# angelocatalani/neural-network-compression

Measured on AMD Instinct MI355X. Metric: weights/sec through prune+k-means (K=256), higher is better.
Workload: dtype f32

## Files before the change

### include/nnc.h

```cpp
#ifndef NNC_H
#define NNC_H

#include <stddef.h>
#include <stdint.h>

#ifdef __cplusplus
extern "C" {
#endif

#define NNC_VERSION 100

#define NNC_OK 0
#define NNC_EINVAL (-1)
#define NNC_ENOSPACE (-2)
#define NNC_EHIP (-3)
#define NNC_ENODEV (-4)

#define NNC_KMAX 1040
#define NNC_CHUNK 8192

int nnc_version(void);
const char *nnc_last_error(void);
int nnc_device_info(char *arch_out, size_t arch_len, int *cu_count_out);

// ... 118 lines not shown

int nnc_kmeans_assign(const float *x, void *ws, const nnc_kmeans_params *p, int which, void *labels_out,
                      int label_bytes, float *quant_out, float *dist_out, int64_t *dist_hist4096_dev, void *stream);

int nnc_topm_hist_f32(const float *d, int64_t n, int32_t shift, int32_t width, int32_t prefix_shift, uint32_t prefix,
                      int64_t *hist4096_dev, void *stream);
int nnc_topm_compact_f32(const float *d, const float *x, int64_t n, uint32_t thr_bits, int64_t *keys_dev,
                         int64_t cap, int64_t *count_dev, void *stream);

int nnc_kmeans_relocate(void *ws, const int64_t *keys_sorted_dev, int32_t nkeys, void *stream);

int nnc_kmeans_reloc_candidates(const float *x_sorted, void *ws, const nnc_kmeans_params *p, int32_t window,
                                float *cand_x_dev, int64_t cap, void *win_dev, int32_t *meta_dev, void *stream);
int nnc_kmeans_relocate_checked(void *ws, const float *cand_x_dev, const float *cand_d_dev, const void *win_dev,
                                const int32_t *meta_dev, int32_t n_empty, int64_t *keys_out_dev, void *stream);
int32_t nnc_kmeans_reloc_window(int64_t n, int32_t n_empty);
size_t nnc_kmeans_reloc_scratch_bytes(int32_t k, int32_t window);
int nnc_kmeans_relocate_windowed(const float *x_sorted, void *ws, const nnc_kmeans_params *p, int32_t n_empty,
                                 void *scratch_dev, size_t scratch_bytes, void *stream);
int nnc_kmeans_reloc_select_local(const float *x_sorted, void *ws, const nnc_kmeans_params *p, int32_t n_empty,
                                  void *scratch_dev, size_t scratch_bytes, int64_t *keys_out_dev, void *stream);
int32_t *nnc_kmeans_reloc_flag(void *ws);
int nnc_kmeans_relocate_if_proven(void *ws, const int64_t *keys_sorted_dev, int32_t nkeys, void *stream);
int nnc_labels_equal(const void *a, const void *b, int64_t n, int label_bytes, int32_t *flag_dev, void *stream);
int nnc_ref_sums_f32(const float *x, int64_t n, float x_mean, const void *labels, int32_t label_bytes, int32_t k,
                     float *sums_out_dev, int64_t *counts_out_dev, void *stream);
int nnc_kmeans_set_done_if(void *ws, const int32_t *flag_dev, int32_t done_code, void *stream);

int nnc_bincount(const void *labels, int label_bytes, int64_t n, int32_t k, int64_t *counts_dev, void *stream);

// ... 343 lines not shown
```

### neural_network_compression_amd/_native.py

```python
from __future__ import annotations

import ctypes
import os

from . import build as _build

c_void_p = ctypes.c_void_p
c_int = ctypes.c_int
c_i32 = ctypes.c_int32
c_i64 = ctypes.c_int64
c_f32 = ctypes.c_float
c_size = ctypes.c_size_t

NNC_OK = 0
NNC_KMAX = 1040
NNC_CHUNK = 8192
FOLD_SUM, FOLD_MEAN, FOLD_STD = 0, 1, 2
NNC_KM_TWO_LAUNCH = 1
NNC_KM_LOOP = 2
NNC_KM_MASS_IN_PLACE = 4
NNC_KM_LOOP_KMAX = 64
CBMM_NONE, CBMM_STREAM, CBMM_TILED, CBMM_BIAS = 0, 1, 2, 3
CBMM_PLAN_LEN = 12
CBMM_PLAN_FIELDS = ("path", "vb", "mt", "copies", "entries", "splits", "rps", "aligned", "lds", "col_tiles", "row_tiles", "workspace")
# ... 126 lines not shown
    "nnc_kmeans_status_async": (c_int, [c_void_p, ctypes.POINTER(KMeansStatus), c_void_p]),
    "nnc_kmeans_status_publish": (c_int, [c_void_p, c_void_p, ctypes.c_uint64, c_void_p]),
    "nnc_kmeans_iterate_publish": (c_int, [c_void_p, c_void_p, ctypes.POINTER(KMeansParams), c_i32, c_void_p, ctypes.c_uint64, c_void_p]),
    "nnc_kmeans_fit": (c_int, [c_void_p, c_void_p, ctypes.POINTER(KMeansParams), c_i32, c_i32, c_void_p, c_size, c_void_p,
                               ctypes.POINTER(ctypes.c_uint64), ctypes.POINTER(KMeansStatus), ctypes.POINTER(c_i32), c_void_p]),
    "nnc_kmeans_fit_sharded": (c_int, [c_void_p, c_void_p, c_void_p, ctypes.POINTER(KMeansParams), ctypes.c_int64, c_i32, c_i32, c_void_p, c_size,
                                       c_void_p, ctypes.POINTER(ctypes.c_uint64), ctypes.POINTER(KMeansStatus), ctypes.POINTER(c_i32), c_void_p]),
    "nnc_kmeans_set_done": (c_int, [c_void_p, c_i32, c_void_p]),
    "nnc_kmeans_label_counts": (c_int, [c_void_p, c_void_p, ctypes.POINTER(KMeansParams), c_int, c_void_p, c_void_p]),
    "nnc_kmeans_get_centers": (c_int, [c_void_p, c_int, c_int, c_void_p, c_void_p]),
    "nnc_kmeans_assign": (c_int, [c_void_p, c_void_p, ctypes.POINTER(KMeansParams), c_int, c_void_p, c_int, c_void_p, c_void_p, c_void_p, c_void_p]),
    "nnc_topm_hist_f32": (c_int, [c_void_p, c_i64, c_i32, c_i32, c_i32, ctypes.c_uint32, c_void_p, c_void_p]),
    "nnc_topm_compact_f32": (c_int, [c_void_p, c_void_p, c_i64, ctypes.c_uint32, c_void_p, c_i64, c_void_p, c_void_p]),
    "nnc_kmeans_relocate": (c_int, [c_void_p, c_void_p, c_i32, c_void_p]),
    "nnc_kmeans_reloc_candidates": (c_int, [c_void_p, c_void_p, ctypes.POINTER(KMeansParams), c_i32, c_void_p, c_i64, c_void_p, c_void_p, c_void_p]),
    "nnc_kmeans_relocate_checked": (c_int, [c_void_p, c_void_p, c_void_p, c_void_p, c_void_p, c_i32, c_void_p, c_void_p]),
    "nnc_kmeans_reloc_window": (c_i32, [c_i64, c_i32]),
    "nnc_kmeans_reloc_scratch_bytes": (c_size, [c_i32, c_i32]),
    "nnc_kmeans_relocate_windowed": (c_int, [c_void_p, c_void_p, ctypes.POINTER(KMeansParams), c_i32, c_void_p, c_size, c_void_p]),
    "nnc_kmeans_reloc_select_local": (c_int, [c_void_p, c_void_p, ctypes.POINTER(KMeansParams), c_i32, c_void_p, c_size, c_void_p, c_void_p]),
    "nnc_kmeans_reloc_flag": (c_void_p, [c_void_p]),
    "nnc_kmeans_relocate_if_proven": (c_int, [c_void_p, c_void_p, c_i32, c_void_p]),
    "nnc_labels_equal": (c_int, [c_void_p, c_void_p, c_i64, c_int, c_void_p, c_void_p]),
    "nnc_ref_sums_f32": (c_int, [c_void_p, c_i64, ctypes.c_float, c_void_p, c_i32, c_i32, c_void_p, c_void_p, c_void_p]),
    "nnc_kmeans_set_done_if": (c_int, [c_void_p, c_void_p, c_i32, c_void_p]),
    "nnc_bincount": (c_int, [c_void_p, c_int, c_i64, c_i32, c_void_p, c_void_p]),
    "nnc_kmeans_fit_reference_f32": (c_int, [c_void_p, c_i32, c_void_p, c_i32, c_i32, c_f32, c_void_p, c_void_p, c_void_p, c_void_p, c_void_p, c_void_p]),
    "nnc_compress_layer_workspace_bytes": (c_size, [c_i64, c_i32]),
    "nnc_compress_layer_host_bytes": (c_size, []),
    "nnc_compress_layer_f32": (c_int, [c_void_p, c_i64, ctypes.POINTER(LayerParams), c_void_p, c_void_p, c_void_p, c_void_p, c_size, c_void_p, c_size,
# ... 182 lines not shown
```

### neural_network_compression_amd/csrc/nnc_hip.hip

```cpp
#include "nnc_common.hpp"
#include "nnc_km_shared.hpp"


extern "C" size_t nnc_kmeans_workspace_bytes(int32_t k)
{
    (void)k;
    return sizeof(KmWs) + 256;
}

extern "C" int32_t nnc_fix_shift(float absmax, int64_t n_total)
{
    int L = 1;
    while (((int64_t)1 << L) < n_total && L < 62) L++;
    if (!(absmax > 0.0f) || !std::isfinite(absmax)) return 0;
    int P = 0;
    (void)std::frexp((double)absmax, &P);
    return std::min(28, 62 - L) - P;
}

__device__ __forceinline__ int fix_f32(float v, int Sft)
{
    return (int)rintf(ldexpf(v, Sft));
}

// ... 2623 lines not shown
#ifndef KM_RELOC_WMIN
#define KM_RELOC_WMIN 64
#endif
#define KM_SURV_MAX 2048
#define KM_SURV_SMALL 384

__device__ __forceinline__ bool km_spec_decide(const KmWs *__restrict__ ws, long long n, int spec_wmax, int *W_out)
{
    const int done = ws->st.done, paused = ws->st.paused, it = ws->st.iter, same = ws->st.same_counts, ne = ws->st.n_empty;
    long long w = KM_RELOC_WMIN;
    while (w < ne) w *= 2;
    if (W_out) *W_out = (int)w;
    return !done && paused == 1 && !(it >= 1 && same) && ne >= 1 && w <= spec_wmax && 2 * w <= n;
}

__device__ __forceinline__ void km_reloc_windows_body(const float *__restrict__ xs, long long n, KmWs *__restrict__ ws, int W, long long cap,
                                                      KmWin *__restrict__ win, int *__restrict__ meta, unsigned *__restrict__ hist0, int spec_wmax)
{
    if (spec_wmax > 0) {
        const bool go = km_spec_decide(ws, n, spec_wmax, &W);
        if (threadIdx.x == 0) ws->spec_go = go ? 1 : 0;
        if (!go) return;
    }
    if (hist0) for (int i = threadIdx.x; i < 4096; i += KM_THREADS) hist0[i] = 0u;
    __shared__ long long bnd[2 * KM_THREADS + 2];
    __shared__ long long wst[2 * KM_THREADS], wen[2 * KM_THREADS];
    __shared__ long long wave_tot[KM_THREADS / 64];
    const int tid = threadIdx.x;
    const KmTab *tab = &ws->tab[ws->cur];
    const int kt = tab->ku, k = ws->p.k;
    const float mean = ws->p.x_mean;
    const int i0 = 2 * tid, i1 = 2 * tid + 1;
    long long a0 = (i0 < kt) ? ws->partials_local[k + tab->orig[i0]] : 0;
    long long a1 = (i1 < kt) ? ws->partials_local[k + tab->orig[i1]] : 0;
    block_scan2<false>(a0, a1, wave_tot);
    if (tid == 0) bnd[0] = 0;
    bnd[i0 + 1] = a0; bnd[i1 + 1] = a1;
    __syncthreads();
    const int nwin = kt + 1;
    const int bad = (bnd[kt] != n) ? 1 : 0;
    if (bad) {
        for (int j = tid; j < nwin; j += KM_THREADS) { KmWin w; w.start = 0; w.len = 0; w.off = 0; win[j] = w; }
        if (tid == 0) { meta[0] = 0; meta[1] = nwin; meta[2] = 1; meta[3] = W; }
        return;
    }
    for (int j = tid; j < 2 * KM_THREADS; j += KM_THREADS) {
        long long st = 0, en = 0;
        if (j < nwin) {
            long long b = bnd[j];
            b = b < 0 ? 0 : (b > n ? n : b);
            long long wl = W, wr = W;
            if (j > 0 && j < kt && n > 0) {
                const double zr = tab->zr[j - 1], zl = tab->zl[j];
                bool more_r = true, more_l = true;
                while (more_r || more_l) {
                    const long long pr = b + wr - 1, pl = b - wl;
                    const float vr = (more_r && pr < n - 1) ? xs[pr] : 0.0f;
                    const float vl = (more_l && pl > 0) ? xs[pl] : 0.0f;
// ... 5 lines not shown
            en = b + wr > n ? n : b + wr;
        }
        wst[j] = st; wen[j] = en;
    }
    __syncthreads();
    long long e0 = wen[i0], e1 = wen[i1];
    block_scan2<true>(e0, e1, wave_tot);
    if (tid == 0) bnd[0] = 0;
    bnd[i0 + 1] = e0; bnd[i1 + 1] = e1;
    __syncthreads();
    long long l0 = 0, l1 = 0, s0 = 0, s1 = 0;
    if (i0 < nwin) { s0 = wst[i0] > bnd[i0] ? wst[i0] : bnd[i0]; l0 = bnd[i0 + 1] - s0; if (l0 <= 0) { l0 = 0; s0 = bnd[i0 + 1]; } }
    if (i1 < nwin) { s1 = wst[i1] > bnd[i1] ? wst[i1] : bnd[i1]; l1 = bnd[i1 + 1] - s1; if (l1 <= 0) { l1 = 0; s1 = bnd[i1 + 1]; } }
    const long long len0 = l0, len1 = l1;
    block_scan2<false>(l0, l1, wave_tot);
    if (i0 < nwin) { KmWin w; w.start = s0; w.len = (int)len0; w.off = l0 <= cap ? (int)(l0 - len0) : 0; win[i0] = w; }
    if (i1 < nwin) { KmWin w; w.start = s1; w.len = (int)len1; w.off = l1 <= cap ? (int)(l1 - len1) : 0; win[i1] = w; }
    if (tid == (nwin - 1) / 2) {
        const long long total = ((nwin - 1) & 1) ? l1 : l0;
        const int over = total > cap ? 1 : 0;
        meta[0] = over ? 0 : (int)total; meta[1] = nwin; meta[2] = bad | over; meta[3] = W;
    }
}

__global__ __launch_bounds__(KM_THREADS) void k_reloc_windows(const float *__restrict__ xs, long long n, KmWs *__restrict__ ws,
                                                              int W, long long cap, KmWin *__restrict__ win, int *__restrict__ meta,
                                                              unsigned *__restrict__ hist0 = nullptr, int spec_wmax = 0)
{
    if (spec_wmax > 0 && threadIdx.x == 0 && km_spec_decide(ws, n, spec_wmax, nullptr)) ws->tab[ws->cur].n_ovf = 0;
    km_reloc_windows_body(xs, n, ws, W, cap, win, meta, hist0, spec_wmax);
}

__global__ __launch_bounds__(KM_THREADS) void k_reloc_head(const float *__restrict__ xs, long long n, KmWs *__restrict__ ws, long long cap,
                                                           KmWin *__restrict__ win, int *__restrict__ meta, unsigned *__restrict__ hist0, int spec_wmax)
{
    if (blockIdx.x == gridDim.x - 1) {
// ... 75 lines not shown
        float xc[1];
        int p[1];
        km_resolve<1>(c, xv, xc, p);
        const float dd = xc[0] - cval_s[p[0]];
        const float dv = dd * dd;
        cand_x[i] = xv[0];
        cand_d[i] = dv;
        atomicAdd(&h0_s[(__float_as_uint(dv) >> 19) & 4095u], 1u);
    }
    __syncthreads();
    for (int i = threadIdx.x; i < 4096; i += KM_THREADS)
        if (h0_s[i]) atomicAdd(&hist0[i], h0_s[i]);
    if (blockIdx.x == 0 && threadIdx.x < 4 && total + threadIdx.x < cap) { cand_x[total + threadIdx.x] = 0.0f; cand_d[total + threadIdx.x] = 0.0f; }
}

__device__ __forceinline__ void km_reloc_select_body(KmWs *__restrict__ ws, const float *__restrict__ cand_x,
                                                     const float *__restrict__ cand_d, const KmWin *__restrict__ win,
                                                     const int *__restrict__ meta, int n_empty, long long *__restrict__ keys_out,
                                                     int do_relocate, const unsigned *__restrict__ hist0, int spec)
{
    if (spec) {
        if (!ws->spec_go) return;
        n_empty = ws->st.n_empty;
    }
    __shared__ __align__(8) unsigned hist[4096];
    __shared__ unsigned long long surv[KM_SURV_MAX];
    __shared__ int wave_i[KM_THREADS / 64];
    __shared__ int s_cut, s_above, s_ge, s_nsurv, s_bad;
    __shared__ KmRelocLds rl;
    __shared__ double zl_s[NNC_KMAX];
    const int tid = threadIdx.x, lane = tid & 63, wv = tid >> 6;
    unsigned long long *strc = NNC_KM_TRACE_PTR;
#define RSTAMP(i) do { if (strc && tid == 0) strc[7000 + (i)] = __builtin_amdgcn_s_memrealtime(); } while (0)
    RSTAMP(0);
    const int n_cand = meta[0];
    const int n_empty_ws = do_relocate ? km_relocate_prepare(ws, &rl) : 0;
    {
        int bad0 = meta[2] ? 1 : 0;
        if (n_empty < 1 || n_cand < n_empty) bad0 |= 2;
        if (bad0) { if (tid == 0) { ws->reloc_fail = bad0; if (spec) ws->st.n_unproven += 1; } return; }
    }
    const int nvec = n_cand >> 2;
    const uint4 *d4 = reinterpret_cast<const uint4 *>(cand_d);
    unsigned prefix = 0, thr = 0;
    int pshift = -1, above = 0, total_ge = n_cand;
    const int shifts[3] = {19, 7, 0}, widths[3] = {12, 12, 7};
    for (int lvl = 0; lvl < 3; lvl++) {
        const int shift = shifts[lvl], width = widths[lvl];
        const unsigned mask = (1u << width) - 1u;
        for (int i = tid; i < 4096; i += KM_THREADS) hist[i] = (lvl == 0 && hist0) ? hist0[i] : 0u;
        if (tid == 0) { s_cut = 0; s_above = above; s_ge = total_ge; }
        __syncthreads();
        const unsigned NOBIN = 0xFFFFu;
        auto bin_of = [&](unsigned u) -> unsigned { return (pshift < 0 || (u >> pshift) == prefix) ? ((u >> shift) & mask) : NOBIN; };
        for (int v0 = 0; v0 < ((lvl == 0 && hist0) ? 0 : nvec); v0 += 8 * KM_THREADS) {
            uint4 qv[8];
#pragma unroll
            for (int u = 0; u < 8; u++) {
                const int v = v0 + u * KM_THREADS + tid;
                qv[u] = v < nvec ? d4[v] : make_uint4(0u, 0u, 0u, 0u);
            }
#pragma unroll
            for (int u = 0; u < 8; u++) {
                const int v = v0 + u * KM_THREADS + tid;
                const bool have = v < nvec;
// ... 158 lines not shown
    __syncthreads();
    RSTAMP(4);
    const int any_bad = s_bad;
    if (tid == 0) { ws->reloc_fail = any_bad; if (spec && any_bad) ws->st.n_unproven += 1; }
    if (any_bad || !do_relocate) return;
    __threadfence_block();
    km_relocate_apply(ws, keys_out, min(m, n_empty + 1), n_empty_ws, &rl);
    if (spec && tid == 0) ws->st.n_relocated += 1;
    RSTAMP(5);
#undef RSTAMP
}

__global__ __launch_bounds__(KM_THREADS) void k_reloc_select(KmWs *__restrict__ ws, const float *__restrict__ cand_x,
                                                             const float *__restrict__ cand_d, const KmWin *__restrict__ win,
                                                             const int *__restrict__ meta, int n_empty, long long *__restrict__ keys_out,
                                                             int do_relocate, const unsigned *__restrict__ hist0, int spec)
{
    km_reloc_select_body(ws, cand_x, cand_d, win, meta, n_empty, keys_out, do_relocate, hist0, spec);
}

__global__ __launch_bounds__(KM_THREADS) void k_reloc_select_finalize(KmWs *__restrict__ ws, const float *__restrict__ cand_x,
                                                                      const float *__restrict__ cand_d, const KmWin *__restrict__ win,
                                                                      const int *__restrict__ meta, long long *__restrict__ keys_out,
                                                                      const unsigned *__restrict__ hist0, nnc_kmeans_status *host_st,
                                                                      unsigned long long *host_ticket, unsigned long long ticket, int lazy)
{
    km_reloc_select_body(ws, cand_x, cand_d, win, meta, 0, keys_out, 1, hist0, 1);
    __syncthreads();
    __builtin_amdgcn_fence(__ATOMIC_ACQUIRE, "agent");
    km_finalize_kernel<KM_THREADS, false, false>(ws, FIN_FROM_PARTIALS, 2, host_st, host_ticket, ticket, lazy, nullptr, 0);
}

static std::atomic<int> g_reloc_dist_attr[NNC_MAX_DEVICES];
static int km_reloc_windows_dist(const float *x_sorted, void *ws, const nnc_kmeans_params *p, int32_t window, float *cand_x,
                                 float *cand_d, int64_t cap, void *win_dev, int32_t *meta_dev, unsigned *hist0, void *stream)
{
    int glog2, rlog2;
    km_defaults(p, &glog2, &rlog2);
    const size_t lds = km_lds_bytes(p->k, glog2, rlog2, false) + (NNC_KMAX + 2) * sizeof(int);
// ... 23 lines not shown
    int rc = km_check(ws, p, "nnc_kmeans_reloc_candidates");
    if (rc) return rc;
    if (!x_sorted || !cand_x_dev || !win_dev || !meta_dev || window < 1) return fail(NNC_EINVAL, "nnc_kmeans_reloc_candidates: bad argument");
    if (cap < 2 * (int64_t)window * (p->k + 1) || cap > 0x7FFFFFFF) return fail(NNC_ENOSPACE, "nnc_kmeans_reloc_candidates: cap must be in [2 * window * (k + 1), 2^31)");
    NNC_LAUNCH_PROF(NNC_PROF_RELOC, k_reloc_windows, dim3(1), dim3(KM_THREADS), 0, S(stream), x_sorted, (long long)p->n,
                       reinterpret_cast<KmWs *>(ws), (int)window, (long long)cap,
                       reinterpret_cast<KmWin *>(win_dev), reinterpret_cast<int *>(meta_dev), (unsigned *)nullptr, 0);
    LAUNCHCHK("k_reloc_windows");
    const int grid = (int)std::min<int64_t>(256, (cap + 16383) / 16384 + p->k / 4 + 1);
    hipLaunchKernelGGL(k_reloc_fill, dim3(grid), dim3(256), 0, S(stream), x_sorted, reinterpret_cast<const KmWin *>(win_dev),
                       reinterpret_cast<const int *>(meta_dev), cand_x_dev, (long long)cap);
    LAUNCHCHK("k_reloc_fill");
    return NNC_OK;
}

#ifdef NNC_DIAG
extern "C" int nnc_debug_reloc_fail(void *ws, int32_t *host_out)
{
    if (!ws || !host_out) return fail(NNC_EINVAL, "nnc_debug_reloc_fail: null pointer");
    HIPCHK(hipMemcpy(host_out, &reinterpret_cast<KmWs *>(ws)->reloc_fail, sizeof(int32_t), hipMemcpyDeviceToHost));
    return NNC_OK;
}
#endif

extern "C" int nnc_kmeans_relocate_checked(void *ws, const float *cand_x_dev, const float *cand_d_dev, const void *win_dev,
                                           const int32_t *meta_dev, int32_t n_empty, int64_t *keys_out_dev, void *stream)
{
    if (!ws || !cand_x_dev || !cand_d_dev || !win_dev || !meta_dev || !keys_out_dev || n_empty < 1 || n_empty > NNC_KMAX)
        return fail(NNC_EINVAL, "nnc_kmeans_relocate_checked: bad argument");
    NNC_LAUNCH_PROF(NNC_PROF_RELOC, k_reloc_select, dim3(1), dim3(KM_THREADS), 0, S(stream), reinterpret_cast<KmWs *>(ws), cand_x_dev, cand_d_dev,
                       reinterpret_cast<const KmWin *>(win_dev), reinterpret_cast<const int *>(meta_dev), (int)n_empty,
                       reinterpret_cast<long long *>(keys_out_dev), 1, (const unsigned *)nullptr, 0);
    LAUNCHCHK("k_reloc_select");
    return NNC_OK;
}


extern "C" int32_t nnc_kmeans_reloc_window(int64_t n, int32_t n_empty)
{
    int64_t w = KM_RELOC_WMIN;
    while (w < n_empty) w *= 2;
    if (n_empty < 1 || w > 1024 || 2 * w > n) return 0;
    return (int32_t)w;
}

static int64_t reloc_cap(int32_t k, int32_t window) { return 8 * (int64_t)window * (k + 1); }

// ... 13 lines not shown
    if (window == 0) return fail(NNC_EINVAL, "nnc_kmeans_relocate_windowed: not applicable (nnc_kmeans_reloc_window() == 0)");
    if (!x_sorted || !scratch_dev || (reinterpret_cast<uintptr_t>(scratch_dev) & 255) != 0)
        return fail(NNC_EINVAL, "nnc_kmeans_relocate_windowed: null or unaligned (256 B) pointer");
    if (scratch_bytes < nnc_kmeans_reloc_scratch_bytes(p->k, window)) return fail(NNC_ENOSPACE, "nnc_kmeans_relocate_windowed: scratch too small");
    const int64_t cap = reloc_cap(p->k, window);
    unsigned char *b = reinterpret_cast<unsigned char *>(scratch_dev);
    float *cand_x = reinterpret_cast<float *>(b); b += reloc_align((size_t)cap * 4);
    float *cand_d = reinterpret_cast<float *>(b); b += reloc_align((size_t)cap * 4);
    void *win = b; b += reloc_align(16 * (size_t)(p->k + 2));
    int32_t *meta = reinterpret_cast<int32_t *>(b); b += reloc_align(16);
    int64_t *keys = reinterpret_cast<int64_t *>(b); b += reloc_align(8 * (size_t)NNC_KMAX);
    unsigned *hist0 = reinterpret_cast<unsigned *>(b);
    if ((rc = km_reloc_windows_dist(x_sorted, ws, p, window, cand_x, cand_d, cap, win, meta, hist0, stream))) return rc;
    NNC_LAUNCH_PROF(NNC_PROF_RELOC, k_reloc_select, dim3(1), dim3(KM_THREADS), 0, S(stream), reinterpret_cast<KmWs *>(ws), cand_x, cand_d,
                       reinterpret_cast<const KmWin *>(win), reinterpret_cast<const int *>(meta), (int)n_empty,
                       reinterpret_cast<long long *>(keys), 1, (const unsigned *)hist0, 0);
    LAUNCHCHK("k_reloc_select");
    return km_launch_finalize(reinterpret_cast<KmWs *>(ws), p, FIN_FROM_PARTIALS, 1, stream);
}

#define KM_SPEC_WMAX 256
static int km_launch_spec_reloc(const float *x_sorted, KmWs *w, const nnc_kmeans_params *p, void *scratch_dev, void *stream,
                                void *host_mapped, uint64_t ticket)
{
    const int32_t wmax = KM_SPEC_WMAX;
    const int64_t cap = reloc_cap(p->k, wmax);
    unsigned char *b = reinterpret_cast<unsigned char *>(scratch_dev);
    float *cand_x = reinterpret_cast<float *>(b); b += reloc_align((size_t)cap * 4);
    float *cand_d = reinterpret_cast<float *>(b); b += reloc_align((size_t)cap * 4);
    KmWin *win = reinterpret_cast<KmWin *>(b); b += reloc_align(16 * (size_t)(p->k + 2));
    int *meta = reinterpret_cast<int *>(b); b += reloc_align(16);
    long long *keys = reinterpret_cast<long long *>(b); b += reloc_align(8 * (size_t)NNC_KMAX);
    unsigned *hist0 = reinterpret_cast<unsigned *>(b);
    int glog2, rlog2;
    km_defaults(p, &glog2, &rlog2);
    const size_t lds = km_lds_bytes(p->k, glog2, rlog2, false) + (NNC_KMAX + 2) * sizeof(int);
    if (lds > 128 * 1024) return fail(NNC_EINVAL, "relocation: search tables too large for the candidate kernel");
    if (!g_reloc_dist_attr[current_device()].load(std::memory_order_acquire)) {
        HIPCHK(hipFuncSetAttribute(reinterpret_cast<const void *>(&k_reloc_dist), hipFuncAttributeMaxDynamicSharedMemorySize, 128 * 1024));
        g_reloc_dist_attr[current_device()].store(1, std::memory_order_release);
    }
    NNC_LAUNCH_PROF(NNC_PROF_RELOC, k_reloc_head, dim3(KM_GMAX / KM_THREADS + 1), dim3(KM_THREADS), 0, S(stream), x_sorted, (long long)p->n, w, (long long)cap, win, meta,
                       hist0, (int)wmax);
    LAUNCHCHK("k_reloc_head");
    const int grid = (int)std::max<int64_t>(1, std::min<int64_t>(128, (2 * (int64_t)64 * (p->k + 1) + KM_THREADS - 1) / KM_THREADS));
    NNC_LAUNCH_PROF(NNC_PROF_RELOC, k_reloc_dist, dim3(grid), dim3(KM_THREADS), lds, S(stream), x_sorted, (const KmWin *)win, (const int *)meta, cand_x, cand_d, (long long)cap,
                       reinterpret_cast<const KmWs *>(w), hist0, 1);
    LAUNCHCHK("k_reloc_dist");
#ifndef KM_CHAIN_FIVE
    if (p->k > 256 && !km_fused(p) && p->prefix_dev) {
        unsigned char *hb = reinterpret_cast<unsigned char *>(host_mapped);
        NNC_LAUNCH_PROF(NNC_PROF_RELOC, k_reloc_select_finalize, dim3(1), dim3(KM_THREADS), 0, S(stream), w, (const float *)cand_x, (const float *)cand_d, (const KmWin *)win,
                        (const int *)meta, keys, (const unsigned *)hist0, reinterpret_cast<nnc_kmeans_status *>(hb),
                        reinterpret_cast<unsigned long long *>(hb ? hb + sizeof(nnc_kmeans_status) : nullptr), (unsigned long long)ticket, 1 | (p->k << 8));
        LAUNCHCHK("k_reloc_select_finalize");
        return NNC_OK;
    }
#endif
    NNC_LAUNCH_PROF(NNC_PROF_RELOC, k_reloc_select, dim3(1), dim3(KM_THREADS), 0, S(stream), w, (const float *)cand_x, (const float *)cand_d, (const KmWin *)win, (const int *)meta, 0, keys, 1, (const unsigned *)hist0, 1);
    LAUNCHCHK("k_reloc_select");
    return km_launch_finalize(w, p, FIN_FROM_PARTIALS, 2, stream, host_mapped, ticket);
}


int nnc_wait_ticket_(void *host_ticket, uint64_t ticket, void *stream)
{
    return km_wait_ticket(reinterpret_cast<volatile unsigned long long *>(host_ticket), (unsigned long long)ticket, S(stream));
}
int km_wait_ticket(volatile unsigned long long *word, unsigned long long ticket, hipStream_t stream)
{
    unsigned long long spins = 0;
    bool synced = false;
    auto t0 = std::chrono::steady_clock::now();
    while (__atomic_load_n(word, __ATOMIC_ACQUIRE) != ticket) {
// ... 25 lines not shown
    unsigned char *hb = reinterpret_cast<unsigned char *>(host_mapped);
    const bool spec_ok = sorted && !one_launch && p.prefix_dev && reloc_scratch_dev && (reinterpret_cast<uintptr_t>(reloc_scratch_dev) & 255) == 0 &&
                         reloc_scratch_bytes >= nnc_kmeans_reloc_scratch_bytes(p.k, KM_SPEC_WMAX) && p.n >= 2 * KM_SPEC_WMAX;
    const bool mass_in_place = (p.flags & NNC_KM_MASS_IN_PLACE) && !lloyd && p.k > 64;
    bool spec = spec_ok && !mass_in_place;
    int batch = one_launch ? p.max_iter : (spec_ok ? 6 : 1);
    if (lloyd) batch = KM_LLOYD_ROUNDS;
    bool first_launch = true;
    int nwin = 0, nrel_seen = status_out->n_relocated, nunp_seen = status_out->n_unproven;
    int nip_seen = status_out->n_in_place;
    int spec_seen = 0, spec_unseen = 0;
    if (!spec_ok) { nrel_seen = 0; nunp_seen = 0; nip_seen = 0; }
    double s_prev = -1.0, s_last = -1.0;
    int i_prev = 0, i_last = 0;
    KmWs *w = reinterpret_cast<KmWs *>(ws);
    for (;;) {
        const uint64_t ticket = ++(*ticket_io);
        unsigned char *sl = hb + (ticket & 1) * slot;
        if (lloyd) {
            if ((rc = km_set_lds_attr())) return rc;
            for (int i = 0; i < batch; i++) {
                const bool last = i == batch - 1;
                if ((rc = km_launch_lloyd_round(x_iter, w, &p, first_launch ? p.max_iter : -1, stream, (last && !spec) ? sl : nullptr, ticket, spec ? 1 : 0))) return rc;
                first_launch = false;
                if (spec && (rc = km_launch_spec_reloc(x_iter, w, &p, reloc_scratch_dev, stream, last ? sl : nullptr, ticket))) return rc;
            }
        } else if (spec) {
            if ((rc = km_set_lds_attr())) return rc;
            const int carry = batch >= 2 ? batch - 2 : batch - 1;
            spec_seen = spec_unseen + carry + 1;
            spec_unseen = batch - 1 - carry;
            for (int i = 0; i < batch; i++) {
                if ((rc = km_launch_accumulate(x_iter, w, &p, stream))) return rc;
// ... 14 lines not shown
        nwin += dev_events;
        nwin += spec_ok ? st.n_unproven - nunp_seen : 0;
        nunp_seen = st.n_unproven;
        if (st.done) break;
        if (lloyd && !st.paused) continue;
        if (spec && !st.paused) {
            if (2 * chain_events > spec_seen) { batch = 4; s_prev = s_last = -1.0; continue; }
            spec = false;
            s_prev = s_last = -1.0;
        }
        if (st.paused) {
            const bool strict_check = st.iter >= 1 && st.same_counts;
            const int32_t window = (sorted && st.paused == 1 && !strict_check) ? nnc_kmeans_reloc_window(p.n, st.n_empty) : 0;
            if (window == 0 || !reloc_scratch_dev || reloc_scratch_bytes < nnc_kmeans_reloc_scratch_bytes(p.k, window)) break;
            if ((rc = nnc_kmeans_relocate_windowed(x_iter, ws, &p, st.n_empty, reloc_scratch_dev, reloc_scratch_bytes, stream))) return rc;
            nwin++;
            if (!lloyd) batch = one_launch ? p.max_iter : 1;
            s_prev = s_last = -1.0;
            continue;
        }
        if (one_launch) continue;
        s_prev = s_last; i_prev = i_last;
        s_last = (double)st.shift_tot; i_last = st.iter;
        batch = std::min(max_batch, batch * 2);
        if (s_prev > 0.0 && s_last > 0.0 && s_prev > s_last && p.tol > 0.0f) {
            const double rate = std::log(s_prev / s_last) / std::max(1, i_last - i_prev);
            const double left = s_last > (double)p.tol ? std::log(s_last / (double)p.tol) / rate : 0.0;
            batch = (int)std::max((double)std::min(max_batch, KM_FIT_LAG + 1), std::min((double)max_batch, std::floor(left * 0.9)));
        }
    }
// ... 9 lines not shown
    const int32_t window = nnc_kmeans_reloc_window(p->n, n_empty);
    if (window == 0) return fail(NNC_EINVAL, "nnc_kmeans_reloc_select_local: not applicable (nnc_kmeans_reloc_window() == 0)");
    if (!x_sorted || !scratch_dev || !keys_out_dev || (reinterpret_cast<uintptr_t>(scratch_dev) & 255) != 0)
        return fail(NNC_EINVAL, "nnc_kmeans_reloc_select_local: null or unaligned (256 B) pointer");
    if (scratch_bytes < nnc_kmeans_reloc_scratch_bytes(p->k, window)) return fail(NNC_ENOSPACE, "nnc_kmeans_reloc_select_local: scratch too small");
    const int64_t cap = reloc_cap(p->k, window);
    unsigned char *b = reinterpret_cast<unsigned char *>(scratch_dev);
    float *cand_x = reinterpret_cast<float *>(b); b += reloc_align((size_t)cap * 4);
    float *cand_d = reinterpret_cast<float *>(b); b += reloc_align((size_t)cap * 4);
    void *win = b; b += reloc_align(16 * (size_t)(p->k + 2));
    int32_t *meta = reinterpret_cast<int32_t *>(b); b += reloc_align(16) + reloc_align(8 * (size_t)NNC_KMAX);
    unsigned *hist0 = reinterpret_cast<unsigned *>(b);
    if ((rc = km_reloc_windows_dist(x_sorted, ws, p, window, cand_x, cand_d, cap, win, meta, hist0, stream))) return rc;
    NNC_LAUNCH_PROF(NNC_PROF_RELOC, k_reloc_select, dim3(1), dim3(KM_THREADS), 0, S(stream), reinterpret_cast<KmWs *>(ws), cand_x, cand_d,
                       reinterpret_cast<const KmWin *>(win), reinterpret_cast<const int *>(meta), (int)n_empty,
                       reinterpret_cast<long long *>(keys_out_dev), 0, (const unsigned *)hist0, 0);
    LAUNCHCHK("k_reloc_select");
    return NNC_OK;
}

extern "C" int32_t *nnc_kmeans_reloc_flag(void *ws)
{
    if (!ws) return nullptr;
    return &reinterpret_cast<KmWs *>(ws)->reloc_fail;
}

__global__ __launch_bounds__(KM_THREADS) void k_relocate_if_proven(KmWs *__restrict__ ws, const long long *__restrict__ keys, int nkeys)
{
    __shared__ KmRelocLds lds;
    if (ws->reloc_fail) return;
    km_relocate_body(ws, keys, nkeys, &lds);
// ... 105 lines not shown
```

Baseline: 10.53 billion.

## Fuse relocation window head and candidate distance kernels into one zoned launch

Replaces the speculative relocation pair k_reloc_head + k_reloc_dist with a single multi-block kernel k_reloc_cand. Each block redundantly recomputes the window table in LDS, labels candidates with a hinted zone binary search, and builds a block-local histogram that it merges into the global one. Because of this, hist0 clearing moves out of the head kernel: the select kernel now zeroes it after consuming it, and a clear kernel runs once before the fit loop. This removes a launch and the dynamic-LDS attribute setup, at the cost of redundant per-block window computation and more complicated histogram-cleanliness invariants.

```diff
diff --git a/include/nnc.h b/include/nnc.h
--- a/include/nnc.h
+++ b/include/nnc.h
@@ -156,6 +156,9 @@
                                 float *cand_x_dev, int64_t cap, void *win_dev, int32_t *meta_dev, void *stream);
 int nnc_kmeans_relocate_checked(void *ws, const float *cand_x_dev, const float *cand_d_dev, const void *win_dev,
                                 const int32_t *meta_dev, int32_t n_empty, int64_t *keys_out_dev, void *stream);
+int nnc_kmeans_reloc_candidates_zoned(const float *x_sorted, void *ws, const nnc_kmeans_params *p, int32_t window, float *cand_x_dev,
+                                      float *cand_d_dev, int64_t cap, void *win_dev, int32_t *meta_dev, uint32_t *hist4096_dev,
+                                      int32_t grid, void *stream);
 int32_t nnc_kmeans_reloc_window(int64_t n, int32_t n_empty);
 size_t nnc_kmeans_reloc_scratch_bytes(int32_t k, int32_t window);
 int nnc_kmeans_relocate_windowed(const float *x_sorted, void *ws, const nnc_kmeans_params *p, int32_t n_empty,
diff --git a/neural_network_compression_amd/_native.py b/neural_network_compression_amd/_native.py
--- a/neural_network_compression_amd/_native.py
+++ b/neural_network_compression_amd/_native.py
@@ -164,6 +164,8 @@
     "nnc_topm_compact_f32": (c_int, [c_void_p, c_void_p, c_i64, ctypes.c_uint32, c_void_p, c_i64, c_void_p, c_void_p]),
     "nnc_kmeans_relocate": (c_int, [c_void_p, c_void_p, c_i32, c_void_p]),
     "nnc_kmeans_reloc_candidates": (c_int, [c_void_p, c_void_p, ctypes.POINTER(KMeansParams), c_i32, c_void_p, c_i64, c_void_p, c_void_p, c_void_p]),
+    "nnc_kmeans_reloc_candidates_zoned": (c_int, [c_void_p, c_void_p, ctypes.POINTER(KMeansParams), c_i32, c_void_p, c_void_p, c_i64, c_void_p, c_void_p,
+                                                  c_void_p, c_i32, c_void_p]),
     "nnc_kmeans_relocate_checked": (c_int, [c_void_p, c_void_p, c_void_p, c_void_p, c_void_p, c_i32, c_void_p, c_void_p]),
     "nnc_kmeans_reloc_window": (c_i32, [c_i64, c_i32]),
     "nnc_kmeans_reloc_scratch_bytes": (c_size, [c_i32, c_i32]),
diff --git a/neural_network_compression_amd/csrc/nnc_hip.hip b/neural_network_compression_amd/csrc/nnc_hip.hip
--- a/neural_network_compression_amd/csrc/nnc_hip.hip
+++ b/neural_network_compression_amd/csrc/nnc_hip.hip
@@ -2661,15 +2661,22 @@
     return !done && paused == 1 && !(it >= 1 && same) && ne >= 1 && w <= spec_wmax && 2 * w <= n;
 }
 
+template <bool LOCAL = false>
 __device__ __forceinline__ void km_reloc_windows_body(const float *__restrict__ xs, long long n, KmWs *__restrict__ ws, int W, long long cap,
-                                                      KmWin *__restrict__ win, int *__restrict__ meta, unsigned *__restrict__ hist0, int spec_wmax)
-{
-    if (spec_wmax > 0) {
+                                                      KmWin *__restrict__ win, int *__restrict__ meta, unsigned *__restrict__ hist0, int spec_wmax,
+                                                      KmWin *win_s = nullptr, int *meta_s = nullptr, bool writer = true)
+{
+    auto put_win = [&](int j, const KmWin &w) { if (LOCAL) win_s[j] = w; if (!LOCAL || writer) win[j] = w; };
+    auto put_meta = [&](int n_cand, int nw, int verdict, int window) {
+        if (LOCAL) { meta_s[0] = n_cand; meta_s[1] = nw; meta_s[2] = verdict; meta_s[3] = window; }
+        if (!LOCAL || writer) { meta[0] = n_cand; meta[1] = nw; meta[2] = verdict; meta[3] = window; }
+    };
+    if (!LOCAL && spec_wmax > 0) {
         const bool go = km_spec_decide(ws, n, spec_wmax, &W);
         if (threadIdx.x == 0) ws->spec_go = go ? 1 : 0;
         if (!go) return;
     }
-    if (hist0) for (int i = threadIdx.x; i < 4096; i += KM_THREADS) hist0[i] = 0u;
+    if (!LOCAL && hist0) for (int i = threadIdx.x; i < 4096; i += KM_THREADS) hist0[i] = 0u;
     __shared__ long long bnd[2 * KM_THREADS + 2];
     __shared__ long long wst[2 * KM_THREADS], wen[2 * KM_THREADS];
     __shared__ long long wave_tot[KM_THREADS / 64];
@@ -2687,8 +2694,8 @@
     const int nwin = kt + 1;
     const int bad = (bnd[kt] != n) ? 1 : 0;
     if (bad) {
-        for (int j = tid; j < nwin; j += KM_THREADS) { KmWin w; w.start = 0; w.len = 0; w.off = 0; win[j] = w; }
-        if (tid == 0) { meta[0] = 0; meta[1] = nwin; meta[2] = 1; meta[3] = W; }
+        for (int j = tid; j < nwin; j += KM_THREADS) { KmWin w; w.start = 0; w.len = 0; w.off = 0; put_win(j, w); }
+        if (tid == 0) put_meta(0, nwin, 1, W);
         return;
     }
     for (int j = tid; j < 2 * KM_THREADS; j += KM_THREADS) {
@@ -2724,12 +2731,12 @@
     if (i1 < nwin) { s1 = wst[i1] > bnd[i1] ? wst[i1] : bnd[i1]; l1 = bnd[i1 + 1] - s1; if (l1 <= 0) { l1 = 0; s1 = bnd[i1 + 1]; } }
     const long long len0 = l0, len1 = l1;
     block_scan2<false>(l0, l1, wave_tot);
-    if (i0 < nwin) { KmWin w; w.start = s0; w.len = (int)len0; w.off = l0 <= cap ? (int)(l0 - len0) : 0; win[i0] = w; }
-    if (i1 < nwin) { KmWin w; w.start = s1; w.len = (int)len1; w.off = l1 <= cap ? (int)(l1 - len1) : 0; win[i1] = w; }
+    if (i0 < nwin) { KmWin w; w.start = s0; w.len = (int)len0; w.off = l0 <= cap ? (int)(l0 - len0) : 0; put_win(i0, w); }
+    if (i1 < nwin) { KmWin w; w.start = s1; w.len = (int)len1; w.off = l1 <= cap ? (int)(l1 - len1) : 0; put_win(i1, w); }
     if (tid == (nwin - 1) / 2) {
         const long long total = ((nwin - 1) & 1) ? l1 : l0;
         const int over = total > cap ? 1 : 0;
-        meta[0] = over ? 0 : (int)total; meta[1] = nwin; meta[2] = bad | over; meta[3] = W;
+        put_meta(over ? 0 : (int)total, nwin, bad | over, W);
     }
 }
 
@@ -2835,10 +2842,115 @@
     if (blockIdx.x == 0 && threadIdx.x < 4 && total + threadIdx.x < cap) { cand_x[total + threadIdx.x] = 0.0f; cand_d[total + threadIdx.x] = 0.0f; }
 }
 
+__device__ __forceinline__ int km_zone_label(const float xc, const int ku, const double *zrm_s, const double *zlm_s, const float2 *cand_s,
+                                             const uint16_t *orig_s, const int hint)
+{
+    const double x = (double)xc;
+    const int ha = max(hint - 2, 0), hb = min(hint + 2, ku - 1);
+    const double ra = zrm_s[max(ha - 1, 0)], rb = zrm_s[hb], la = zlm_s[ha], lb = zlm_s[min(hb + 1, ku - 1)];
+    int l = (ha > 0 && ra < x) ? ha : 0, h = (rb >= x) ? hb : ku - 1;
+    while (l < h) { const int m = (l + h) >> 1; if (zrm_s[m] >= x) h = m; else l = m + 1; }
+    int plo = l;
+    l = (la <= x) ? ha : 0; h = (hb < ku - 1 && lb > x) ? hb : ku - 1;
+    while (l < h) { const int m = (l + h + 1) >> 1; if (zlm_s[m] <= x) l = m; else h = m - 1; }
+    int phi = l;
+    if (phi < plo) { plo = 0; phi = ku - 1; }
+    const float2 c0 = cand_s[plo];
+    float bestd = c0.y + (-2.0f * (xc * c0.x));
+    int best = plo;
+    for (int q = plo + 1; q <= phi; q++) {
+        const float2 cq = cand_s[q];
+        const float d = cq.y + (-2.0f * (xc * cq.x));
+        if (d < bestd || (d == bestd && orig_s[q] < orig_s[best])) { bestd = d; best = q; }
+    }
+    return best;
+}
+
+__global__ __launch_bounds__(KM_THREADS) void k_reloc_cand(const float *__restrict__ xs, long long n, KmWs *__restrict__ ws, int W, long long cap,
+                                                           KmWin *__restrict__ win, int *__restrict__ meta, float *__restrict__ cand_x,
+                                                           float *__restrict__ cand_d, unsigned *__restrict__ hist0, int spec_wmax)
+{
+    __shared__ KmWin win_s[NNC_KMAX + 2];
+    __shared__ int meta_s[4];
+    __shared__ double zrm_s[NNC_KMAX], zlm_s[NNC_KMAX];
+    __shared__ float2 cand_s[NNC_KMAX];
+    __shared__ uint16_t orig_s[NNC_KMAX];
+    __shared__ unsigned h0_s[4096];
+    __shared__ double zscan_s[2 * (KM_THREADS / 64)];
+    const int tid = threadIdx.x;
+    const bool writer = blockIdx.x == 0;
+    if (spec_wmax > 0) {
+        const bool go = km_spec_decide(ws, n, spec_wmax, &W);
+        if (writer && tid == 0) ws->spec_go = go ? 1 : 0;
+        if (!go) return;
+    }
+    const KmTab *__restrict__ tab = &ws->tab[ws->cur];
+    const int ku = tab->ku;
+    const float mean = ws->p.x_mean;
+    for (int q = tid; q < ku; q += KM_THREADS) { zrm_s[q] = tab->zr[q]; zlm_s[q] = tab->zl[q]; cand_s[q] = tab->cand[q]; orig_s[q] = tab->orig[q]; }
+    for (int i = tid; i < 4096; i += KM_THREADS) h0_s[i] = 0u;
+    km_reloc_windows_body<true>(xs, n, ws, W, cap, win, meta, nullptr, 0, win_s, meta_s, writer);
+    __syncthreads();
+    const long long total = meta_s[0];
+    const int nwin = meta_s[1];
+    if (meta_s[2]) {
+        if (writer && tid < 4 && tid < cap) { cand_x[tid] = 0.0f; cand_d[tid] = 0.0f; }
+        return;
+    }
+    int in_order = 1;
+    for (int q = tid; q + 1 < ku; q += KM_THREADS) in_order &= (zrm_s[q + 1] >= zrm_s[q]) && (zlm_s[q] <= zlm_s[q + 1]);
+    if (!__syncthreads_and(in_order)) {
+        const int lane = tid & 63, wv = tid >> 6;
+        const int i0 = 2 * tid, i1 = i0 + 1;
+        const int j0 = ku - 1 - 2 * tid, j1 = j0 - 1;
+        const double a0 = i0 < ku ? zrm_s[i0] : -INFINITY, a1 = fmax(a0, i1 < ku ? zrm_s[i1] : -INFINITY);
+        const double b0 = j0 >= 0 ? zlm_s[j0] : INFINITY, b1 = fmin(b0, j1 >= 0 ? zlm_s[j1] : INFINITY);
+        double sa = a1, sb = b1;
+        for (int off = 1; off < 64; off <<= 1) {
+            const double ta = __shfl_up(sa, off), tb = __shfl_up(sb, off);
+            if (lane >= off) { sa = fmax(sa, ta); sb = fmin(sb, tb); }
+        }
+        if (lane == 63) { zscan_s[wv] = sa; zscan_s[KM_THREADS / 64 + wv] = sb; }
+        __syncthreads();
+        double pa = -INFINITY, pb = INFINITY;
+        for (int w = 0; w < wv; w++) { pa = fmax(pa, zscan_s[w]); pb = fmin(pb, zscan_s[KM_THREADS / 64 + w]); }
+        const double qa = __shfl_up(sa, 1), qb = __shfl_up(sb, 1);
+        if (lane > 0) { pa = fmax(pa, qa); pb = fmin(pb, qb); }
+        if (i0 < ku) zrm_s[i0] = fmax(pa, a0);
+        if (i1 < ku) zrm_s[i1] = fmax(pa, a1);
+        if (j0 >= 0) zlm_s[j0] = fmin(pb, b0);
+        if (j1 >= 0) zlm_s[j1] = fmin(pb, b1);
+        __syncthreads();
+    }
+    for (long long i = (long long)blockIdx.x * KM_THREADS + tid; i < total; i += (long long)gridDim.x * KM_THREADS) {
+        int l = 0, h = nwin - 1;
+        while (l < h) { const int m = (l + h + 1) >> 1; if (win_s[m].off <= (int)i) l = m; else h = m - 1; }
+        KmWin w = win_s[l];
+        while (w.len == 0 || (int)i - w.off >= w.len) { l--; w = win_s[l]; }
+        const float x = xs[w.start + ((int)i - w.off)];
+        const float xc = x - mean;
+        const int p = km_zone_label(xc, ku, zrm_s, zlm_s, cand_s, orig_s, min(l, ku - 1));
+        const float dd = xc - cand_s[p].x;
+        const float dv = dd * dd;
+        cand_x[i] = x;
+        cand_d[i] = dv;
+        atomicAdd(&h0_s[(__float_as_uint(dv) >> 19) & 4095u], 1u);
+    }
+    __syncthreads();
+    for (int i = tid; i < 4096; i += KM_THREADS)
+        if (h0_s[i]) atomicAdd(&hist0[i], h0_s[i]);
+    if (writer && tid < 4 && total + tid < cap) { cand_x[total + tid] = 0.0f; cand_d[total + tid] = 0.0f; }
+}
+
+__global__ __launch_bounds__(KM_THREADS) void k_spec_hist_clear(unsigned *__restrict__ hist0)
+{
+    hist0[blockIdx.x * KM_THREADS + threadIdx.x] = 0u;
+}
+
 __device__ __forceinline__ void km_reloc_select_body(KmWs *__restrict__ ws, const float *__restrict__ cand_x,
                                                      const float *__restrict__ cand_d, const KmWin *__restrict__ win,
                                                      const int *__restrict__ meta, int n_empty, long long *__restrict__ keys_out,
-                                                     int do_relocate, const unsigned *__restrict__ hist0, int spec)
+                                                     int do_relocate, unsigned *__restrict__ hist0, int spec)
 {
     if (spec) {
         if (!ws->spec_go) return;
@@ -2859,7 +2971,11 @@
     {
         int bad0 = meta[2] ? 1 : 0;
         if (n_empty < 1 || n_cand < n_empty) bad0 |= 2;
-        if (bad0) { if (tid == 0) { ws->reloc_fail = bad0; if (spec) ws->st.n_unproven += 1; } return; }
+        if (bad0) {
+            if (hist0 && !(bad0 & 1)) for (int i = tid; i < 4096; i += KM_THREADS) hist0[i] = 0u;
+            if (tid == 0) { ws->reloc_fail = bad0; if (spec) ws->st.n_unproven += 1; }
+            return;
+        }
     }
     const int nvec = n_cand >> 2;
     const uint4 *d4 = reinterpret_cast<const uint4 *>(cand_d);
@@ -2869,7 +2985,10 @@
     for (int lvl = 0; lvl < 3; lvl++) {
         const int shift = shifts[lvl], width = widths[lvl];
         const unsigned mask = (1u << width) - 1u;
-        for (int i = tid; i < 4096; i += KM_THREADS) hist[i] = (lvl == 0 && hist0) ? hist0[i] : 0u;
+        for (int i = tid; i < 4096; i += KM_THREADS) {
+            hist[i] = (lvl == 0 && hist0) ? hist0[i] : 0u;
+            if (lvl == 0 && hist0) hist0[i] = 0u;
+        }
         if (tid == 0) { s_cut = 0; s_above = above; s_ge = total_ge; }
         __syncthreads();
         const unsigned NOBIN = 0xFFFFu;
@@ -3058,7 +3177,7 @@
 __global__ __launch_bounds__(KM_THREADS) void k_reloc_select(KmWs *__restrict__ ws, const float *__restrict__ cand_x,
                                                              const float *__restrict__ cand_d, const KmWin *__restrict__ win,
                                                              const int *__restrict__ meta, int n_empty, long long *__restrict__ keys_out,
-                                                             int do_relocate, const unsigned *__restrict__ hist0, int spec)
+                                                             int do_relocate, unsigned *__restrict__ hist0, int spec)
 {
     km_reloc_select_body(ws, cand_x, cand_d, win, meta, n_empty, keys_out, do_relocate, hist0, spec);
 }
@@ -3066,7 +3185,7 @@
 __global__ __launch_bounds__(KM_THREADS) void k_reloc_select_finalize(KmWs *__restrict__ ws, const float *__restrict__ cand_x,
                                                                       const float *__restrict__ cand_d, const KmWin *__restrict__ win,
                                                                       const int *__restrict__ meta, long long *__restrict__ keys_out,
-                                                                      const unsigned *__restrict__ hist0, nnc_kmeans_status *host_st,
+                                                                      unsigned *__restrict__ hist0, nnc_kmeans_status *host_st,
                                                                       unsigned long long *host_ticket, unsigned long long ticket, int lazy)
 {
     km_reloc_select_body(ws, cand_x, cand_d, win, meta, 0, keys_out, 1, hist0, 1);
@@ -3120,6 +3239,22 @@
     return NNC_OK;
 }
 
+extern "C" int nnc_kmeans_reloc_candidates_zoned(const float *x_sorted, void *ws, const nnc_kmeans_params *p, int32_t window, float *cand_x_dev,
+                                                 float *cand_d_dev, int64_t cap, void *win_dev, int32_t *meta_dev, uint32_t *hist4096_dev,
+                                                 int32_t grid, void *stream)
+{
+    int rc = km_check(ws, p, "nnc_kmeans_reloc_candidates_zoned");
+    if (rc) return rc;
+    if (!x_sorted || !cand_x_dev || !cand_d_dev || !win_dev || !meta_dev || !hist4096_dev || window < 1 || grid < 0 || grid > 1024)
+        return fail(NNC_EINVAL, "nnc_kmeans_reloc_candidates_zoned: bad argument");
+    if (cap < 2 * (int64_t)window * (p->k + 1) || cap > 0x7FFFFFFF) return fail(NNC_ENOSPACE, "nnc_kmeans_reloc_candidates_zoned: cap must be in [2 * window * (k + 1), 2^31)");
+    if (grid == 0) grid = (int)std::max<int64_t>(1, std::min<int64_t>(128, (2 * (int64_t)64 * (p->k + 1) + KM_THREADS - 1) / KM_THREADS));
+    NNC_LAUNCH_PROF(NNC_PROF_RELOC, k_reloc_cand, dim3(grid), dim3(KM_THREADS), 0, S(stream), x_sorted, (long long)p->n, reinterpret_cast<KmWs *>(ws), (int)window,
+                       (long long)cap, reinterpret_cast<KmWin *>(win_dev), reinterpret_cast<int *>(meta_dev), cand_x_dev, cand_d_dev, reinterpret_cast<unsigned *>(hist4096_dev), 0);
+    LAUNCHCHK("k_reloc_cand");
+    return NNC_OK;
+}
+
 #ifdef NNC_DIAG
 extern "C" int nnc_debug_reloc_fail(void *ws, int32_t *host_out)
 {
@@ -3136,7 +3271,7 @@
         return fail(NNC_EINVAL, "nnc_kmeans_relocate_checked: bad argument");
     NNC_LAUNCH_PROF(NNC_PROF_RELOC, k_reloc_select, dim3(1), dim3(KM_THREADS), 0, S(stream), reinterpret_cast<KmWs *>(ws), cand_x_dev, cand_d_dev,
                        reinterpret_cast<const KmWin *>(win_dev), reinterpret_cast<const int *>(meta_dev), (int)n_empty,
-                       reinterpret_cast<long long *>(keys_out_dev), 1, (const unsigned *)nullptr, 0);
+                       reinterpret_cast<long long *>(keys_out_dev), 1, (unsigned *)nullptr, 0);
     LAUNCHCHK("k_reloc_select");
     return NNC_OK;
 }
@@ -3180,12 +3315,24 @@
     if ((rc = km_reloc_windows_dist(x_sorted, ws, p, window, cand_x, cand_d, cap, win, meta, hist0, stream))) return rc;
     NNC_LAUNCH_PROF(NNC_PROF_RELOC, k_reloc_select, dim3(1), dim3(KM_THREADS), 0, S(stream), reinterpret_cast<KmWs *>(ws), cand_x, cand_d,
                        reinterpret_cast<const KmWin *>(win), reinterpret_cast<const int *>(meta), (int)n_empty,
-                       reinterpret_cast<long long *>(keys), 1, (const unsigned *)hist0, 0);
+                       reinterpret_cast<long long *>(keys), 1, hist0, 0);
     LAUNCHCHK("k_reloc_select");
     return km_launch_finalize(reinterpret_cast<KmWs *>(ws), p, FIN_FROM_PARTIALS, 1, stream);
 }
 
 #define KM_SPEC_WMAX 256
+static unsigned *km_spec_hist0(void *scratch_dev, int32_t k)
+{
+    const size_t cap = (size_t)reloc_cap(k, KM_SPEC_WMAX);
+    return reinterpret_cast<unsigned *>(reinterpret_cast<unsigned char *>(scratch_dev) + 2 * reloc_align(cap * 4) + reloc_align(16 * (size_t)(k + 2)) +
+                                        reloc_align(16) + reloc_align(8 * (size_t)NNC_KMAX));
+}
+static int km_spec_hist_clear(void *scratch_dev, int32_t k, void *stream)
+{
+    hipLaunchKernelGGL(k_spec_hist_clear, dim3(4096 / KM_THREADS), dim3(KM_THREADS), 0, S(stream), km_spec_hist0(scratch_dev, k));
+    LAUNCHCHK("k_spec_hist_clear");
+    return NNC_OK;
+}
 static int km_launch_spec_reloc(const float *x_sorted, KmWs *w, const nnc_kmeans_params *p, void *scratch_dev, void *stream,
                                 void *host_mapped, uint64_t ticket)
 {
@@ -3196,34 +3343,23 @@
     float *cand_d = reinterpret_cast<float *>(b); b += reloc_align((size_t)cap * 4);
     KmWin *win = reinterpret_cast<KmWin *>(b); b += reloc_align(16 * (size_t)(p->k + 2));
     int *meta = reinterpret_cast<int *>(b); b += reloc_align(16);
-    long long *keys = reinterpret_cast<long long *>(b); b += reloc_align(8 * (size_t)NNC_KMAX);
-    unsigned *hist0 = reinterpret_cast<unsigned *>(b);
-    int glog2, rlog2;
-    km_defaults(p, &glog2, &rlog2);
-    const size_t lds = km_lds_bytes(p->k, glog2, rlog2, false) + (NNC_KMAX + 2) * sizeof(int);
-    if (lds > 128 * 1024) return fail(NNC_EINVAL, "relocation: search tables too large for the candidate kernel");
-    if (!g_reloc_dist_attr[current_device()].load(std::memory_order_acquire)) {
-        HIPCHK(hipFuncSetAttribute(reinterpret_cast<const void *>(&k_reloc_dist), hipFuncAttributeMaxDynamicSharedMemorySize, 128 * 1024));
-        g_reloc_dist_attr[current_device()].store(1, std::memory_order_release);
-    }
-    NNC_LAUNCH_PROF(NNC_PROF_RELOC, k_reloc_head, dim3(KM_GMAX / KM_THREADS + 1), dim3(KM_THREADS), 0, S(stream), x_sorted, (long long)p->n, w, (long long)cap, win, meta,
+    long long *keys = reinterpret_cast<long long *>(b);
+    unsigned *hist0 = km_spec_hist0(scratch_dev, p->k);
+    const int grid = (int)std::max<int64_t>(1, std::min<int64_t>(128, (2 * (int64_t)64 * (p->k + 1) + KM_THREADS - 1) / KM_THREADS));
+    NNC_LAUNCH_PROF(NNC_PROF_RELOC, k_reloc_cand, dim3(grid), dim3(KM_THREADS), 0, S(stream), x_sorted, (long long)p->n, w, 0, (long long)cap, win, meta, cand_x, cand_d,
                        hist0, (int)wmax);
-    LAUNCHCHK("k_reloc_head");
-    const int grid = (int)std::max<int64_t>(1, std::min<int64_t>(128, (2 * (int64_t)64 * (p->k + 1) + KM_THREADS - 1) / KM_THREADS));
-    NNC_LAUNCH_PROF(NNC_PROF_RELOC, k_reloc_dist, dim3(grid), dim3(KM_THREADS), lds, S(stream), x_sorted, (const KmWin *)win, (const int *)meta, cand_x, cand_d, (long long)cap,
-                       reinterpret_cast<const KmWs *>(w), hist0, 1);
-    LAUNCHCHK("k_reloc_dist");
+    LAUNCHCHK("k_reloc_cand");
 #ifndef KM_CHAIN_FIVE
     if (p->k > 256 && !km_fused(p) && p->prefix_dev) {
         unsigned char *hb = reinterpret_cast<unsigned char *>(host_mapped);
         NNC_LAUNCH_PROF(NNC_PROF_RELOC, k_reloc_select_finalize, dim3(1), dim3(KM_THREADS), 0, S(stream), w, (const float *)cand_x, (const float *)cand_d, (const KmWin *)win,
-                        (const int *)meta, keys, (const unsigned *)hist0, reinterpret_cast<nnc_kmeans_status *>(hb),
+                        (const int *)meta, keys, hist0, reinterpret_cast<nnc_kmeans_status *>(hb),
                         reinterpret_cast<unsigned long long *>(hb ? hb + sizeof(nnc_kmeans_status) : nullptr), (unsigned long long)ticket, 1 | (p->k << 8));
         LAUNCHCHK("k_reloc_select_finalize");
         return NNC_OK;
     }
 #endif
-    NNC_LAUNCH_PROF(NNC_PROF_RELOC, k_reloc_select, dim3(1), dim3(KM_THREADS), 0, S(stream), w, (const float *)cand_x, (const float *)cand_d, (const KmWin *)win, (const int *)meta, 0, keys, 1, (const unsigned *)hist0, 1);
+    NNC_LAUNCH_PROF(NNC_PROF_RELOC, k_reloc_select, dim3(1), dim3(KM_THREADS), 0, S(stream), w, (const float *)cand_x, (const float *)cand_d, (const KmWin *)win, (const int *)meta, 0, keys, 1, hist0, 1);
     LAUNCHCHK("k_reloc_select");
     return km_launch_finalize(w, p, FIN_FROM_PARTIALS, 2, stream, host_mapped, ticket);
 }
@@ -3279,9 +3415,14 @@
     double s_prev = -1.0, s_last = -1.0;
     int i_prev = 0, i_last = 0;
     KmWs *w = reinterpret_cast<KmWs *>(ws);
+    bool hist_clean = false;
     for (;;) {
         const uint64_t ticket = ++(*ticket_io);
         unsigned char *sl = hb + (ticket & 1) * slot;
+        if (spec && !hist_clean) {
+            if ((rc = km_spec_hist_clear(reloc_scratch_dev, p.k, stream))) return rc;
+            hist_clean = true;
+        }
         if (lloyd) {
             if ((rc = km_set_lds_attr())) return rc;
             for (int i = 0; i < batch; i++) {
@@ -3326,6 +3467,7 @@
             const int32_t window = (sorted && st.paused == 1 && !strict_check) ? nnc_kmeans_reloc_window(p.n, st.n_empty) : 0;
             if (window == 0 || !reloc_scratch_dev || reloc_scratch_bytes < nnc_kmeans_reloc_scratch_bytes(p.k, window)) break;
             if ((rc = nnc_kmeans_relocate_windowed(x_iter, ws, &p, st.n_empty, reloc_scratch_dev, reloc_scratch_bytes, stream))) return rc;
+            hist_clean = false;
             nwin++;
             if (!lloyd) batch = one_launch ? p.max_iter : 1;
             s_prev = s_last = -1.0;
@@ -3365,7 +3507,7 @@
     if ((rc = km_reloc_windows_dist(x_sorted, ws, p, window, cand_x, cand_d, cap, win, meta, hist0, stream))) return rc;
     NNC_LAUNCH_PROF(NNC_PROF_RELOC, k_reloc_select, dim3(1), dim3(KM_THREADS), 0, S(stream), reinterpret_cast<KmWs *>(ws), cand_x, cand_d,
                        reinterpret_cast<const KmWin *>(win), reinterpret_cast<const int *>(meta), (int)n_empty,
-                       reinterpret_cast<long long *>(keys_out_dev), 0, (const unsigned *)hist0, 0);
+                       reinterpret_cast<long long *>(keys_out_dev), 0, hist0, 0);
     LAUNCHCHK("k_reloc_select");
     return NNC_OK;
 }
```

Result: no change. 10.51 billion (-0.2%).
